# vliu15/speech-masters-thesis

Hardware: AMD Instinct MI355X
Metric: LJSpeech utterances/sec per VQ-VAE train step (higher is better)
Workload: dtype bf16

## Files before the change

speech-masters-thesis_amd/csrc/conv_common.h:

```cpp
#pragma once
#include <algorithm>
#include <cstdlib>

#include "smt_common.h"

namespace smt {

typedef __bf16 bf16x8 __attribute__((ext_vector_type(8)));
typedef __bf16 bf16x4 __attribute__((ext_vector_type(4)));
typedef short s16x4 __attribute__((ext_vector_type(4)));

__device__ __forceinline__ unsigned fmix32(unsigned h) {
  h ^= h >> 16; h *= 0x85EBCA6Bu; h ^= h >> 13; h *= 0xC2B2AE35u; h ^= h >> 16;
  return h;
}
__device__ __forceinline__ bool drop_keep(unsigned long long i, unsigned key, unsigned thresh16) {
  unsigned h = fmix32((unsigned)(i >> 1) * 0x9E3779B1u + key);
  unsigned bits = (h >> (16 * (unsigned)(i & 1))) & 0xFFFFu;
  return bits >= thresh16;
}

template <typename T> struct Tr;
template <> struct Tr<__bf16> {
  static constexpr int EPV = 8;
  static constexpr int CCH = 128;
  static constexpr int KC = 128;
  static constexpr int BM = 128;
};
template <> struct Tr<float> {
  static constexpr int EPV = 4;
  static constexpr int CCH = 64;
  static constexpr int KC = 64;
  static constexpr int BM = 64;
};

template <typename T, int EPV> struct Vec { T v[EPV]; } __attribute__((aligned(16)));

__device__ __forceinline__ unsigned pack_bf16x2(float lo, float hi) {
  typedef __bf16 bf16x2 __attribute__((ext_vector_type(2)));
  bf16x2 v = {(__bf16)lo, (__bf16)hi};
  return __builtin_bit_cast(unsigned, v);
}

typedef short s16x2v __attribute__((ext_vector_type(2)));
typedef unsigned short u16x2v __attribute__((ext_vector_type(2)));
__device__ __forceinline__ unsigned pk_relu_bf16(unsigned w) {
  return __builtin_bit_cast(unsigned, __builtin_elementwise_max(__builtin_bit_cast(s16x2v, w), s16x2v{0, 0}));
}
__device__ __forceinline__ unsigned pk_keep_mask(unsigned h, unsigned thr_m1) {
  u16x2v d = __builtin_elementwise_sub_sat(__builtin_bit_cast(u16x2v, h), __builtin_bit_cast(u16x2v, thr_m1));
  d = __builtin_elementwise_min(d, u16x2v{1, 1});
  return __builtin_bit_cast(unsigned, (u16x2v)(u16x2v{0, 0} - d));
}

__device__ __forceinline__ float gate_tanh(float x) {
  const float e = __builtin_amdgcn_exp2f(x * 2.885390081777927f);
  return 1.f - 2.f * __builtin_amdgcn_rcpf(e + 1.f);
}

__device__ __forceinline__ void lds_dma16(const void* gsrc, void* lds_dst_wave_base) {
  __builtin_amdgcn_global_load_lds((const void __attribute__((address_space(1)))*)gsrc,
                                   (void __attribute__((address_space(3)))*)lds_dst_wave_base, 16, 0, 0);
}

typedef int i32x4v __attribute__((ext_vector_type(4)));
__device__ __forceinline__ __amdgpu_buffer_rsrc_t ws_rsrc(const void* base, long long byte_off, unsigned bytes) {
  return __builtin_amdgcn_make_buffer_rsrc(const_cast<char*>(reinterpret_cast<const char*>(base)) + byte_off, 0, (int)bytes, 0x00020000);
}
__device__ __forceinline__ void ws_dma16(__amdgpu_buffer_rsrc_t rs, unsigned voff, void* lds_wave_base) {
  __builtin_amdgcn_raw_ptr_buffer_load_lds(rs, (__attribute__((address_space(3))) void*)lds_wave_base, 16, (int)voff, 0, 0, 0);
}
__device__ __forceinline__ bool wg_tile_run(int ntiles, int tiles_per_wg, int& wg, int& tile_begin, int& tile_end) {
  const int nwg = gridDim.x;
  wg = (blockIdx.x & 7) * (nwg >> 3) + (blockIdx.x >> 3);
  tile_begin = wg * tiles_per_wg;
  tile_end = min(ntiles, tile_begin + tiles_per_wg);
  return tile_begin < tile_end;
}

__device__ __forceinline__ void pair_up8(unsigned (&v)[8]) {
#pragma unroll
  for (int h2 = 0; h2 < 2; ++h2)
#pragma unroll
    for (int d = 0; d < 2; ++d) {
      auto sw = __builtin_amdgcn_permlane32_swap(v[4 * h2 + d], v[4 * h2 + 2 + d], false, false);
      v[4 * h2 + d] = sw[0]; v[4 * h2 + 2 + d] = sw[1];
    }
}
__device__ __forceinline__ void store_paired(const unsigned (&v)[8], __amdgpu_buffer_rsrc_t rs, unsigned vo) {
  __builtin_amdgcn_raw_buffer_store_b128(i32x4v{(int)v[0], (int)v[1], (int)v[2], (int)v[3]}, rs, (int)vo, 0, 0);
  __builtin_amdgcn_raw_buffer_store_b128(i32x4v{(int)v[4], (int)v[5], (int)v[6], (int)v[7]}, rs, (int)(vo + 32u), 0, 0);
}

struct UntrackedRsrc { i32x4v w; };
__device__ __forceinline__ UntrackedRsrc untracked_rsrc(const void* base, long long byte_off, unsigned bytes) {
  const unsigned long long a = reinterpret_cast<unsigned long long>(base) + (unsigned long long)byte_off;
  UntrackedRsrc r;
  r.w = i32x4v{__builtin_amdgcn_readfirstlane((int)(unsigned)a), __builtin_amdgcn_readfirstlane((int)((a >> 32) & 0xffffu)),
               __builtin_amdgcn_readfirstlane((int)bytes), 0x00020000};
  return r;
}
__device__ __forceinline__ void untracked_dma16(const UntrackedRsrc& rs, unsigned voff, const void* lds_wave_base) {
  const unsigned m0v = __builtin_amdgcn_readfirstlane(
      (int)(unsigned)reinterpret_cast<size_t>((__attribute__((address_space(3))) const void*)lds_wave_base));
  asm volatile("s_mov_b32 m0, %2\n\ts_nop 4\n\tbuffer_load_dwordx4 %0, %1, 0 offen lds" : : "v"(voff), "s"(rs.w), "s"(m0v) : "memory");
}

__device__ __forceinline__ i32x4v untracked_load16(const void* sbase, unsigned voff) {
  i32x4v v;
  asm volatile("s_nop 4\n\tglobal_load_dwordx4 %0, %1, %2" : "=v"(v) : "v"(voff), "s"(sbase) : "memory");
  return v;
}

typedef unsigned u32x2v __attribute__((ext_vector_type(2)));
__device__ __forceinline__ u32x2v untracked_load8(const void* sbase, unsigned voff) {
  u32x2v v;
  asm volatile("s_nop 4\n\tglobal_load_dwordx2 %0, %1, %2" : "=v"(v) : "v"(voff), "s"(sbase) : "memory");
  return v;
}

template <typename T> __device__ __forceinline__ void pin_v(T& x) { asm volatile("" : "+v"(x)); }
template <typename T, int N> __device__ __forceinline__ void pin_v(T (&a)[N]) {
#pragma unroll
  for (int i = 0; i < N; ++i) pin_v(a[i]);
}
template <int N, typename... R> __device__ __forceinline__ void vm_wait(R&... regs) {
  static_assert(0 <= N && N <= 63, "vmcnt is a 6-bit field on gfx9");
  asm volatile("s_waitcnt vmcnt(%0)" ::"n"(N) : "memory");
  (pin_v(regs), ...);
}
template <int N, typename... R> __device__ __forceinline__ void lgkm_wait(R&... regs) {
  static_assert(0 <= N && N <= 15, "lgkmcnt is a 4-bit field on gfx9");
  asm volatile("s_waitcnt lgkmcnt(%0)" ::"n"(N) : "memory");
  (pin_v(regs), ...);
}
template <int N, typename... R> __device__ __forceinline__ void vm_wait_or_drain(bool counted, R&... regs) {
  if (counted) vm_wait<N>();
  else vm_wait<0>();
  (pin_v(regs), ...);
}
template <int N, typename... R> __device__ __forceinline__ void step_end_wait(R&... regs) {
  __builtin_amdgcn_sched_barrier(0);
  vm_wait<N>(regs...);
}

__device__ __forceinline__ int scalar_load_i32(const int* ptr) {
  int v;
  asm volatile("s_nop 4\n\ts_load_dword %0, %1, 0x0\n\ts_waitcnt lgkmcnt(0)" : "=s"(v) : "s"(ptr) : "memory");
  return v;
}

struct ConvArgs {
  const void* x; const void* w; const float* bias; void* y; const void* res; const void* gate_h; void* y_act;
  const int* lens_in; const int* lens_out;
  long long x_bs, y_bs, res_bs, gh_bs, ya_bs;
  int ldx, ldy, ldr, ldgh, ldya;
  int B, Tin, Tout, Cin, Cout;
  int taps, stride, dil, pad;
  int out_stride, out_offset, Ty;
  int act_out, epi_act;
  unsigned drop_keys[8]; int site_width; unsigned drop_thresh16; float drop_scale;
  const unsigned* drop_keys_dev; int drop_keys_dev_stride;
  int tiles_per_batch;
  int rs;
  const void* x2; const void* w2; const float* bias2; const int* lens_in2; long long x2_bs; int ldx2;
  int dbg;
};

__device__ __forceinline__ unsigned site_key(const ConvArgs& p, int site) {
  return p.drop_keys_dev ? p.drop_keys_dev[(site & 7) * p.drop_keys_dev_stride] : p.drop_keys[site & 7];
}

struct WsPlan { int buf_bytes; size_t lds; int tiles_per_wg; dim3 grid; };
bool plan_conv_ws(ConvArgs& p, WsPlan& pl);
// ... 19 lines not shown
```

speech-masters-thesis_amd/csrc/conv_ws.hip:

```cpp
#include <algorithm>
#include <cstdlib>
#include <type_traits>

#include "smt_common.h"
#include "conv_common.h"

namespace smt {

#ifndef SMT_WS_STAMP
#define SMT_WS_STAMP 0
#endif
#if SMT_WS_STAMP
__device__ unsigned long long ws_dbg[256 * 8 * 8];
#define WS_T(var) const unsigned long long var = __builtin_readcyclecounter()
#define WS_ACC(k, a, b) do { if (lane == 0 && wg < 256) ws_dbg[(wg * 8 + wave) * 8 + (k)] += (b) - (a); } while (0)
#else
#define WS_T(var) do {} while (0)
#define WS_ACC(k, a, b) do {} while (0)
#endif
constexpr int WS_AGPR_TAPS = 8;
constexpr int WS_BM = 128, WS_BN = 128, WS_NT = 256, WS_EPI = 128 * 256;
constexpr int WS_KC = 128, WS_ROWB = WS_KC * 2, WS_KSTEPS = WS_KC / 16;

template <int I, int N, typename F>
__device__ __forceinline__ void static_for(F&& f) {
  if constexpr (I < N) {
    f(std::integral_constant<int, I>{});
    static_for<I + 1, N>(f);
  }
}


__device__ __forceinline__ bf16x8 ws_wfrag(const unsigned char* wrow, int kk, int hh, int co) {
  return *reinterpret_cast<const bf16x8*>(wrow + (((2 * kk + hh) ^ (co & 15)) << 4));
}

__device__ __forceinline__ void ws_decode(int tiles_per_batch, int rs, int tile, int& b, int& cls, int& t0) {
  const int bb = tile / tiles_per_batch;
  b = bb / rs; cls = bb - b * rs;
  t0 = (tile - bb * tiles_per_batch) * WS_BM;
}

__device__ __forceinline__ unsigned ws_tap_base(unsigned abase, int ar, int hh) { return abase + ar * WS_ROWB + ((hh ^ (ar & 15)) << 4); }
template <int NTAPS>
__device__ __forceinline__ unsigned ws_frag_addr(const unsigned (&tap_base)[NTAPS], int q) {
  return tap_base[q / WS_KSTEPS] ^ (32u * (q % WS_KSTEPS));
}

template <int MW>
__device__ __forceinline__ void ws_read_frags(bf16x8 (&afr)[MW], unsigned ap) {
#pragma unroll
  for (int i = 0; i < MW; ++i)
    asm volatile("ds_read_b128 %0, %1 offset:%2" : "=v"(afr[i]) : "v"(ap), "n"(i * 32 * WS_ROWB));
}
__device__ __forceinline__ void ws_first_use(f32x16& acc) { asm volatile("s_nop 4" : "+v"(acc)); }
__device__ __forceinline__ void ws_first_use(f32x16& acc0, f32x16& acc1) { asm volatile("s_nop 4" : "+v"(acc0), "+v"(acc1)); }
__device__ __forceinline__ void ws_mfma(f32x16& acc, const bf16x8& w, const bf16x8& a, bool w_in_agpr) {
  if (w_in_agpr) asm volatile("v_mfma_f32_32x32x16_bf16 %0, %1, %2, %0" : "+v"(acc) : "a"(w), "v"(a));
  else asm volatile("v_mfma_f32_32x32x16_bf16 %0, %1, %2, %0" : "+v"(acc) : "v"(w), "v"(a));
}
template <int MW>
__device__ __forceinline__ void ws_drain(f32x16 (&acc)[MW]) {
  static_assert(MW == 2 || MW == 4, "the drain names two or four accumulators");
#define WS_DRAIN_NOPS "s_nop 15\n\ts_nop 15\n\ts_nop 15\n\ts_nop 15"
  if constexpr (MW == 4) asm volatile(WS_DRAIN_NOPS : "+v"(acc[0]), "+v"(acc[1]), "+v"(acc[2]), "+v"(acc[3]));
  else asm volatile(WS_DRAIN_NOPS : "+v"(acc[0]), "+v"(acc[1]));
#undef WS_DRAIN_NOPS
}

template <int NTAPS, int MODE>
__global__ __launch_bounds__(WS_NT) void conv_ws_kernel(ConvArgs p, const __bf16* __restrict__ zero_page,
                                                        int tiles_per_wg, int buf_bytes) {
  const bool has_y = MODE == 0 ? (p.y != nullptr) : (MODE == 2);
  const bool has_act_out = MODE == 0 ? (p.act_out != 0) : (MODE == 1);
  const bool has_res = MODE == 0 ? (p.res != nullptr) : (MODE == 2);
  const bool has_epi_act = MODE == 0 ? (p.epi_act != 0) : (MODE == 2);
  typedef __bf16 T;
  constexpr int BM = WS_BM, BN = WS_BN, KC = WS_KC, NT = WS_NT, MW = BM / 32, ROWB = WS_ROWB;
  extern __shared__ __attribute__((aligned(1024))) unsigned char smem[];
  const int tid = threadIdx.x, lane = tid & 63, wave = tid >> 6;
  const int r = lane & 31, hh = lane >> 5;
  const int lrow = lane >> 4, lch = lane & 15;
  const int n0 = blockIdx.y * BN;
  const int rs = p.rs;

  int wg, tile_begin, tile_end;
  if (!wg_tile_run(p.tiles_per_batch * p.B * rs, tiles_per_wg, wg, tile_begin, tile_end)) return;

  unsigned char* lds_res = smem + 2 * (size_t)buf_bytes + wave * (WS_EPI / 4);
  unsigned char* lds_act = lds_res + WS_EPI;
  const unsigned lds_base = (unsigned)(uintptr_t)(__attribute__((address_space(3))) unsigned char*)smem;

  bf16x8 wfrag[NTAPS][KC / 16];
  {
    const int co = n0 + wave * 32 + r;
#pragma unroll
    for (int s = 0; s < NTAPS; ++s) {
      const unsigned char* wrow = reinterpret_cast<const unsigned char*>(p.w) + ((size_t)s * p.Cout + co) * ROWB;
#pragma unroll
      for (int kk = 0; kk < KC / 16; ++kk)
        wfrag[s][kk] = ws_wfrag(wrow, kk, hh, co);
    }
  }
  const int col0 = n0 + wave * 32 + 4 * hh;
  float bval[16];
// ... 135 lines not shown
        uint2 uv[4], rv[4];
#pragma unroll
        for (int g = 0; g < 4; ++g) {
          const int eoff = row * 64 + ((g ^ swz) << 4) + 8 * hh;
          uv[g] = *reinterpret_cast<const uint2*>(lds_act + eoff);
          rv[g] = *reinterpret_cast<const uint2*>(lds_res + eoff);
        }
        unsigned yp[8];
#pragma unroll
        for (int g = 0; g < 4; ++g) {
          const unsigned uvp[2] = {uv[g].x, uv[g].y}, rvp[2] = {rv[g].x, rv[g].y};
#pragma unroll
          for (int j = 0; j < 2; ++j) {
            const unsigned ypk = pack_bf16x2(acc[i][4 * g + 2 * j] + bval[4 * g + 2 * j], acc[i][4 * g + 2 * j + 1] + bval[4 * g + 2 * j + 1]);
            const float o0 = __builtin_bit_cast(float, ypk << 16), o1 = __builtin_bit_cast(float, ypk & 0xffff0000u);
            const float v0 = (uvp[j] & 0x7fffu) ? o0 * srow : 0.f, v1 = (uvp[j] & 0x7fff0000u) ? o1 * srow : 0.f;
            yp[2 * g + j] = pack_bf16x2(v0 + __builtin_bit_cast(float, rvp[j] << 16), v1 + __builtin_bit_cast(float, rvp[j] & 0xffff0000u));
          }
        }
        pair_up8(yp);
        store_paired(yp, ry, (unsigned)tc * pitch_y + (unsigned)hh * 16u);
      }
    } else {
#pragma unroll
    for (int i = 0; i < MW; ++i) {
      const int row = 32 * i + r;
      const int tc = t0 + row;
      const int ty = cls + rs * tc;
      const float keep_row = (ty >= len_out) ? 0.f : 1.f;
      const int swz = (row >> 2) & 3;
      unsigned yp[8], up[8];
      {
#pragma unroll
      for (int g = 0; g < 4; ++g) {
        float o[4];
#pragma unroll
        for (int k = 0; k < 4; ++k) o[k] = (float)(T)(acc[i][4 * g + k] + bval[4 * g + k]);
        const int eoff = row * 64 + ((g ^ swz) << 4) + 8 * hh;
        if (has_epi_act) {
          const bf16x4 uv = *reinterpret_cast<const bf16x4*>(lds_act + eoff);
#pragma unroll
          for (int k = 0; k < 4; ++k) o[k] = ((float)uv[k] != 0.f) ? o[k] * p.drop_scale : 0.f;
        }
        if (has_res) {
          const bf16x4 rv = *reinterpret_cast<const bf16x4*>(lds_res + eoff);
#pragma unroll
          for (int k = 0; k < 4; ++k) o[k] = fmaf(o[k], keep_row, (float)rv[k]);
        } else {
#pragma unroll
          for (int k = 0; k < 4; ++k) o[k] *= keep_row;
        }
        yp[2 * g] = pack_bf16x2(o[0], o[1]);
        yp[2 * g + 1] = pack_bf16x2(o[2], o[3]);
        if (has_act_out) {
          const int col = col0 + 8 * g;
          const int site = col / p.site_width;
          const unsigned key = site_key(p, site);
          const unsigned long long base = ((unsigned long long)b * p.Ty + ty) * p.site_width + (col - site * p.site_width);
#pragma unroll
          for (int k = 0; k < 4; k += 2) {
            const unsigned h = fmix32((unsigned)((base + k) >> 1) * 0x9E3779B1u + key);
            const bool k0 = (h & 0xFFFFu) >= p.drop_thresh16, k1 = (h >> 16) >= p.drop_thresh16;
            up[2 * g + (k >> 1)] = pack_bf16x2((k0 && o[k] > 0.f) ? o[k] * p.drop_scale : 0.f,
                                               (k1 && o[k + 1] > 0.f) ? o[k + 1] * p.drop_scale : 0.f);
          }
        }
      }
      }
      if (has_y) {
        pair_up8(yp);
        store_paired(yp, ry, (unsigned)tc * pitch_y + (unsigned)hh * 16u);
      }
      if (has_act_out) {
        pair_up8(up);
        store_paired(up, ru, (unsigned)tc * pitch_u + (unsigned)hh * 16u);
      }
    }
    }
    WS_T(c7);
    WS_ACC(0, c0, c1); WS_ACC(1, c1, c2); WS_ACC(3, c2, c4); WS_ACC(4, c4, c5); WS_ACC(5, c5, c6); WS_ACC(6, c6, c7); WS_ACC(7, c0, c0 + 1);
  }
}

template <int NTAPS>
__global__ __launch_bounds__(WS_NT) void conv_ws_pipe_kernel(ConvArgs p, const __bf16* __restrict__ zero_page,
                                                             int tiles_per_wg, int buf_bytes) {
  constexpr int BM = WS_BM, BN = WS_BN, KC = WS_KC, NT = WS_NT, MW = BM / 32, ROWB = WS_ROWB;
  constexpr int NSTEP = NTAPS * (KC / 16), NGAP = NSTEP * MW;
  constexpr int PH_UNIT = 12, PH_ROW = 4 * PH_UNIT + 2, PH_TILE = MW * PH_ROW;
  constexpr int AGPR_TAPS = NTAPS < 8 ? NTAPS : 8;
  static_assert(MW == 4, "four accumulators");
  extern __shared__ __attribute__((aligned(1024))) unsigned char smem[];
  const int tid = threadIdx.x, lane = tid & 63, wave = tid >> 6;
  const int r = lane & 31, hh = lane >> 5;
  const int lrow = lane >> 4, lch = lane & 15;
  const int n0 = blockIdx.y * BN;
  const int rs = p.rs;

  int wg, tile_begin, tile_end;
  if (!wg_tile_run(p.tiles_per_batch * p.B * rs, tiles_per_wg, wg, tile_begin, tile_end)) return;
  const unsigned lds_base = (unsigned)(uintptr_t)(__attribute__((address_space(3))) unsigned char*)smem;

  bf16x8 wfrag[NTAPS][KC / 16];
  {
    const int co = n0 + wave * 32 + r;
#pragma unroll
    for (int s = 0; s < NTAPS; ++s) {
      const unsigned char* wrow = reinterpret_cast<const unsigned char*>(p.w) + ((size_t)s * p.Cout + co) * ROWB;
#pragma unroll
      for (int kk = 0; kk < KC / 16; ++kk)
        wfrag[s][kk] = ws_wfrag(wrow, kk, hh, co);
    }
  }
  const int col0 = n0 + wave * 32 + 4 * hh;
  float bval[16];
#pragma unroll
  for (int e = 0; e < 16; ++e) bval[e] = p.bias ? p.bias[col0 + 8 * (e >> 2) + (e & 3)] : 0.f;
  unsigned keyg[4], cshalf[4];
#pragma unroll
  for (int g = 0; g < 4; ++g) {
    const int col = col0 + 8 * g;
    const int site = col / p.site_width;
    keyg[g] = site_key(p, site);
    cshalf[g] = (unsigned)(col - site * p.site_width) >> 1;
  }
  const int rows_in = BM + (NTAPS - 1) * p.dil;
  const int rows_pad = (rows_in + 3) & ~3;

  auto decode = [&](int tile, int& b, int& cls, int& t0) { ws_decode(p.tiles_per_batch, rs, tile, b, cls, t0); };
  const unsigned pitch_x = (unsigned)p.ldx * rs * 2u;
  const unsigned voff_a0 = (unsigned)(4 * wave + lrow) * pitch_x + (unsigned)((lch ^ ((4 * wave + lrow) & 15)) << 4);
  const int ngroups = rows_pad >> 2;
  auto stage_a = [&](int tile, int buf) {
    int b, cls, t0;
    decode(tile, b, cls, t0);
    const int len_full = p.lens_in ? min(scalar_load_i32(p.lens_in + b), p.Tin) : p.Tin;
    const int len_in = max(0, (len_full - cls + rs - 1) / rs);
    const __amdgpu_buffer_rsrc_t rx = ws_rsrc(p.x, ((long long)b * p.x_bs + (long long)cls * p.ldx) * 2, (unsigned)len_in * pitch_x);
    unsigned vo = voff_a0 + (unsigned)(t0 - p.pad) * pitch_x;
    unsigned char* dst = smem + (size_t)buf * buf_bytes + wave * 1024;
    for (int g = wave; g < ngroups; g += NT / 64) {
      ws_dma16(rx, vo, dst);
      vo += 16u * pitch_x; dst += 4096;
    }
  };

  unsigned pc[MW][8];
  int p_b = 0, p_cls = 0, p_t0 = 0, p_Tc = 0, p_len = 0;
  __amdgpu_buffer_rsrc_t p_ru = ws_rsrc(p.y_act, 0, 0);
  float o0 = 0.f, o1 = 0.f, o2 = 0.f, o3 = 0.f, u0 = 0.f, u1 = 0.f, u2 = 0.f, u3 = 0.f, keepf = 1.f;
  unsigned h0 = 0, h1 = 0, rh = 0, up[8];
  int ty = 0;
  auto fbits = [](unsigned v) { return __builtin_bit_cast(float, v); };
  auto epi = [&](auto M) {
    constexpr int m = decltype(M)::value;
    constexpr int i = m / PH_ROW, rem = m % PH_ROW;
    if constexpr (rem < 4 * PH_UNIT) {
      constexpr int g = rem / PH_UNIT, ph = rem % PH_UNIT;
      if constexpr (ph == 0) {
        if constexpr (g == 0) {
          const int tc = p_t0 + 32 * i + r;
          ty = (tc < p_Tc) ? p_cls + rs * tc : -1;
          keepf = (ty >= p_len) ? 0.f : 1.f;
          rh = (unsigned)((((unsigned long long)p_b * p.Ty + (unsigned)max(ty, 0)) * (unsigned)p.site_width) >> 1);
        }
      } else if constexpr (ph == 1) {
        o0 = fbits(pc[i][2 * g] << 16) * keepf; o1 = fbits(pc[i][2 * g] & 0xffff0000u) * keepf;
      } else if constexpr (ph == 2) {
        o2 = fbits(pc[i][2 * g + 1] << 16) * keepf; o3 = fbits(pc[i][2 * g + 1] & 0xffff0000u) * keepf;
      } else if constexpr (ph == 3) {
        h0 = (rh + cshalf[g]) * 0x9E3779B1u + keyg[g]; h1 = h0 + 0x9E3779B1u;
      } else if constexpr (ph == 4) {
        h0 ^= h0 >> 16; h0 *= 0x85EBCA6Bu; h1 ^= h1 >> 16; h1 *= 0x85EBCA6Bu;
      } else if constexpr (ph == 5) {
        h0 ^= h0 >> 13; h0 *= 0xC2B2AE35u; h1 ^= h1 >> 13; h1 *= 0xC2B2AE35u;
      } else if constexpr (ph == 6) {
        h0 ^= h0 >> 16; h1 ^= h1 >> 16;
      } else if constexpr (ph == 7) {
        u0 = ((h0 & 0xFFFFu) >= p.drop_thresh16 && o0 > 0.f) ? o0 * p.drop_scale : 0.f;
      } else if constexpr (ph == 8) {
        u1 = ((h0 >> 16) >= p.drop_thresh16 && o1 > 0.f) ? o1 * p.drop_scale : 0.f;
      } else if constexpr (ph == 9) {
        u2 = ((h1 & 0xFFFFu) >= p.drop_thresh16 && o2 > 0.f) ? o2 * p.drop_scale : 0.f;
      } else if constexpr (ph == 10) {
        u3 = ((h1 >> 16) >= p.drop_thresh16 && o3 > 0.f) ? o3 * p.drop_scale : 0.f;
      } else {
        up[2 * g] = pack_bf16x2(u0, u1); up[2 * g + 1] = pack_bf16x2(u2, u3);
      }
    } else if constexpr (rem == 4 * PH_UNIT) {
      pair_up8(up);
    } else {
      if (ty >= 0) {
        store_paired(up, p_ru, (unsigned)ty * ((unsigned)p.ldya * 2u) + (unsigned)hh * 16u);
      }
    }
  };

  stage_a(tile_begin, 0);
  vm_wait<0>();
  const int wave_s = __builtin_amdgcn_readfirstlane(wave);
#pragma unroll
  for (int i = 0; i < MW; ++i)
#pragma unroll
    for (int e = 0; e < 8; ++e) pc[i][e] = 0;
  for (int tile = tile_begin; tile < tile_end; ++tile) {
    const int buf = (tile - tile_begin) & 1;
    int b, cls, t0;
    decode(tile, b, cls, t0);
    WS_T(c0);
    __syncthreads();
    WS_T(c1);
    __amdgpu_buffer_rsrc_t rx_n = ws_rsrc(p.x, 0, 0);
    unsigned vo_in = 0;
    int n_in = 0;
    if (tile + 1 < tile_end) {
      int nb, ncls, nt0;
      decode(tile + 1, nb, ncls, nt0);
      const int len_full = p.lens_in ? min(scalar_load_i32(p.lens_in + nb), p.Tin) : p.Tin;
      const int len_in = max(0, (len_full - ncls + rs - 1) / rs);
      rx_n = ws_rsrc(p.x, ((long long)nb * p.x_bs + (long long)ncls * p.ldx) * 2, (unsigned)len_in * pitch_x);
      vo_in = voff_a0 + (unsigned)(nt0 - p.pad) * pitch_x;
      n_in = ngroups;
    }
    unsigned char* const dst_in = smem + (size_t)(buf ^ 1) * buf_bytes + wave_s * 1024;
    constexpr int WS_IN_SLOTS = 12, WS_IN_EVERY = 2;
    static_assert(WS_IN_SLOTS * WS_IN_EVERY <= NSTEP, "the pieces fit the tap loop");
    WS_T(c2);

    f32x16 acc[MW];
#pragma unroll
    for (int i = 0; i < MW; ++i)
#pragma unroll
      for (int e = 0; e < 16; ++e) acc[i][e] = 0.f;
    const unsigned abase = lds_base + (unsigned)buf * (unsigned)buf_bytes;
    unsigned tap_base[NTAPS];
#pragma unroll
    for (int s = 0; s < NTAPS; ++s) tap_base[s] = ws_tap_base(abase, r + s * p.dil, hh);
    auto frag_addr = [&](int q) -> unsigned { return ws_frag_addr(tap_base, q); };
    bf16x8 afr[2][MW];

    ws_read_frags(afr[0], frag_addr(0));
    static_for<0, NSTEP>([&](auto Q) {
      constexpr int q = decltype(Q)::value;
      if constexpr (q + 1 < NSTEP) {
        ws_read_frags(afr[(q + 1) & 1], frag_addr(q + 1));
        lgkm_wait<MW>();
      } else {
        lgkm_wait<0>();
      }
      static_for<0, MW>([&](auto I) {
        constexpr int i = decltype(I)::value;
        if constexpr (q == 0) ws_first_use(acc[i]);
        ws_mfma(acc[i], wfrag[q / (KC / 16)][q % (KC / 16)], afr[q & 1][i], q / (KC / 16) < AGPR_TAPS);
        if constexpr (i == 0 && q % WS_IN_EVERY == 0 && q / WS_IN_EVERY < WS_IN_SLOTS) {
          constexpr int j = q / WS_IN_EVERY;
          __builtin_amdgcn_sched_barrier(0);
          if (wave_s + 4 * j < n_in) ws_dma16(rx_n, vo_in + (unsigned)(16 * j) * pitch_x, dst_in + j * 4096);
          __builtin_amdgcn_sched_barrier(0);
        }
        if constexpr (4 * q + i < PH_TILE) {
          __builtin_amdgcn_sched_barrier(0);
          epi(std::integral_constant<int, 4 * q + i>{});
          __builtin_amdgcn_sched_barrier(0);
        }
      });
    });
    static_for<(NGAP < PH_TILE ? NGAP : PH_TILE), PH_TILE>(epi);
    ws_drain(acc);
    WS_T(c5);
    vm_wait<0>();
    WS_T(c6);
#pragma unroll
    for (int i = 0; i < MW; ++i)
#pragma unroll
      for (int e = 0; e < 16; e += 2) pc[i][e >> 1] = pack_bf16x2(acc[i][e] + bval[e], acc[i][e + 1] + bval[e + 1]);
    p_b = b; p_cls = cls; p_t0 = t0;
    p_ru = ws_rsrc(p.y_act, ((long long)b * p.ya_bs + n0 + wave_s * 32) * 2, (unsigned)p.Ty * ((unsigned)p.ldya * 2u));
    p_Tc = (p.Tout - cls + rs - 1) / rs;
    p_len = p.lens_out ? scalar_load_i32(p.lens_out + b) : 0x7fffffff;
    WS_T(c7);
    WS_ACC(0, c0, c1); WS_ACC(1, c1, c2); WS_ACC(4, c2, c5); WS_ACC(5, c5, c6); WS_ACC(6, c6, c7); WS_ACC(7, c0, c0 + 1);
  }
  static_for<0, PH_TILE>(epi);
}

constexpr int WS2_NT = 512;
constexpr int WS2_MAX_TAPS = 3;

template <int NTAPS, int MODE>
__global__ __launch_bounds__(WS2_NT) void conv_ws2_kernel(ConvArgs p, const __bf16* __restrict__ zero_page,
                                                          int tiles_per_wg, int buf_bytes) {
  constexpr int BM = WS_BM, BN = WS_BN, KC = WS_KC, MW = 2, ROWB = WS_ROWB;
  constexpr int NSTEP = NTAPS * (KC / 16), NG = 5;
  static_assert(MODE == 1 || MODE == 2, "two epilogues");
  constexpr int AGPR_TAPS = NTAPS < 4 ? NTAPS : 4;
  static_assert(NTAPS <= 5, "weights of more than five taps do not fit two waves per SIMD");
  extern __shared__ __attribute__((aligned(1024))) unsigned char smem[];
  const int tid = threadIdx.x, lane = tid & 63;
  const int wave = __builtin_amdgcn_readfirstlane(tid >> 6);
  const int cw = wave & 3, rhalf = wave >> 2;
  const int r = lane & 31, hh = lane >> 5;
  const int n0 = blockIdx.y * BN;
  const int rs = p.rs;

  int wg, tile_begin, tile_end;
  if (!wg_tile_run(p.tiles_per_batch * p.B * rs, tiles_per_wg, wg, tile_begin, tile_end)) return;

  float* lds_bias = reinterpret_cast<float*>(smem + 2 * (size_t)buf_bytes);
  unsigned char* lds_res = smem + 2 * (size_t)buf_bytes + 1024 + wave * (WS_EPI / 8);
  unsigned char* lds_act = lds_res + WS_EPI;
  const unsigned lds_base = (unsigned)(uintptr_t)(__attribute__((address_space(3))) unsigned char*)smem;
  if (tid < BN) lds_bias[tid] = p.bias ? p.bias[n0 + tid] : 0.f;

  bf16x8 wfrag[NTAPS][KC / 16];
  {
    const int co = n0 + cw * 32 + r;
#pragma unroll
    for (int s = 0; s < NTAPS; ++s) {
      const unsigned char* wrow = reinterpret_cast<const unsigned char*>(p.w) + ((size_t)s * p.Cout + co) * ROWB;
#pragma unroll
      for (int kk = 0; kk < KC / 16; ++kk)
        wfrag[s][kk] = ws_wfrag(wrow, kk, hh, co);
    }
  }
  const int col0 = n0 + cw * 32 + 4 * hh;
  const unsigned HC = 0x9E3779B1u;
  const unsigned swh = (unsigned)p.site_width >> 1;
  unsigned kc[4];
  unsigned rowh_lane = 0;
  const unsigned thr_m1 = (p.drop_thresh16 - 1u) * 0x00010001u;
  if (MODE == 1) {
#pragma unroll
    for (int g = 0; g < 4; ++g) {
      const int col = col0 + 8 * g;
      const int site = col / p.site_width;
      kc[g] = ((unsigned)(col - site * p.site_width) >> 1) * HC + site_key(p, site);
    }
    rowh_lane = HC * swh * (unsigned)(rs * r);
  }
  const int rows_in = BM + (NTAPS - 1) * p.dil;
  const int ngroups = (rows_in + 3) >> 2;

  const unsigned pitch_x = (unsigned)p.ldx * rs * 2u;
  unsigned voff_a[NG];
#pragma unroll
  for (int j = 0; j < NG; ++j) {
    const int row = 4 * (wave + 8 * j) + (lane >> 4);
    voff_a[j] = (unsigned)row * pitch_x + (unsigned)(((lane & 15) ^ (row & 15)) << 4);
  }
  const unsigned pitch_o = (MODE == 2 ? (unsigned)p.ldy : (unsigned)p.ldya) * rs * 2u;
  const unsigned voff_o = (unsigned)(64 * rhalf + r) * pitch_o + (unsigned)hh * 16u;
  const unsigned pitch_r = (unsigned)p.ldr * rs * 2u, pitch_g = (unsigned)p.ldgh * rs * 2u;
  const int elr = 64 * rhalf + (lane >> 2);
  const unsigned echunk = (unsigned)(((lane & 3) ^ ((lane >> 4) & 3)) << 4);

  auto decode = [&](int tile, int& b, int& cls, int& t0) { ws_decode(p.tiles_per_batch, rs, tile, b, cls, t0); };
  auto stage_a = [&](int tile, int buf) {
    int b, cls, t0;
    decode(tile, b, cls, t0);
    const int len_full = p.lens_in ? min(scalar_load_i32(p.lens_in + b), p.Tin) : p.Tin;
    const int len_in = max(0, (len_full - cls + rs - 1) / rs);
// ... 68 lines not shown
  vm_wait<0>();
  int pb = 0, pcls = 0, pt0 = 0, pTc = 0;
  for (int tile = tile_begin; tile < tile_end; ++tile) {
    const int buf = (tile - tile_begin) & 1;
    int b, cls, t0;
    decode(tile, b, cls, t0);
    const int Tc = (p.Tout - cls + rs - 1) / rs;
    WS_T(c0);
    __syncthreads();
    WS_T(c1);
    if (tile + 1 < tile_end) stage_a(tile + 1, buf ^ 1);
    WS_T(c2);
    if (rhalf == 1 && tile > tile_begin) epilogue(pb, pcls, pt0, pTc);
    WS_T(c3);
    if (MODE == 2) {
      stage_epi(p.res, p.res_bs, p.ldr, pitch_r, b, cls, t0, Tc, lds_res);
      stage_epi(p.gate_h, p.gh_bs, p.ldgh, pitch_g, b, cls, t0, Tc, lds_act);
    }
    WS_T(c4);
#pragma unroll
    for (int i = 0; i < MW; ++i)
#pragma unroll
      for (int e = 0; e < 16; ++e) acc[i][e] = 0.f;
    const unsigned abase = lds_base + (unsigned)buf * (unsigned)buf_bytes + (unsigned)(64 * rhalf) * ROWB;
    unsigned tap_base[NTAPS];
#pragma unroll
    for (int s = 0; s < NTAPS; ++s) {
      const int ar = r + s * p.dil;
      tap_base[s] = abase + ar * ROWB + ((hh ^ (ar & 15)) << 4);
    }
    auto frag_addr = [&](int q) -> unsigned { return ws_frag_addr(tap_base, q); };
    bf16x8 afr[3][MW];
#pragma unroll
    for (int q0 = 0; q0 < 2; ++q0) {
      const unsigned ap = frag_addr(q0);
      ws_read_frags(afr[q0], ap);
    }
    static_for<0, NSTEP>([&](auto Q) {
      constexpr int q = decltype(Q)::value;
      if constexpr (q + 2 < NSTEP) {
        const unsigned ap = frag_addr(q + 2);
        ws_read_frags(afr[(q + 2) % 3], ap);
        lgkm_wait<2 * MW>();
      } else if constexpr (q + 1 < NSTEP) {
        lgkm_wait<MW>();
      } else {
        lgkm_wait<0>();
      }
      static_assert(MW == 2, "two accumulators per wave");
      if constexpr (q == 0) ws_first_use(acc[0], acc[1]);
      ws_mfma(acc[0], wfrag[q / (KC / 16)][q % (KC / 16)], afr[q % 3][0], q / (KC / 16) < AGPR_TAPS);
      ws_mfma(acc[1], wfrag[q / (KC / 16)][q % (KC / 16)], afr[q % 3][1], q / (KC / 16) < AGPR_TAPS);
    });
    ws_drain(acc);
    WS_T(c5);
    vm_wait<0>();
    WS_T(c6);
    if (rhalf == 0) epilogue(b, cls, t0, Tc);
    WS_T(c7);
    WS_ACC(0, c0, c1); WS_ACC(1, c1, c2); WS_ACC(2, c2, c3); WS_ACC(3, c3, c4); WS_ACC(4, c4, c5); WS_ACC(5, c5, c6);
    WS_ACC(6, c6, c7); WS_ACC(7, c0, c0 + 1);
    pb = b; pcls = cls; pt0 = t0; pTc = Tc;
  }
  if (rhalf == 1) epilogue(pb, pcls, pt0, pTc);
}

#ifndef SMT_WS_AB
#define SMT_WS_AB 0
#endif

static int ws_min_tiles() {
  static const int v = getenv("SMT_WS_MIN_TILES") ? atoi(getenv("SMT_WS_MIN_TILES")) : 512;
  return v;
}

bool plan_conv_ws(ConvArgs& p, WsPlan& pl) {
  static const bool no_ws = getenv("SMT_CONV_NO_WS") != nullptr;
  const int tc_max = (p.Tout + p.rs - 1) / p.rs;
  const int rows_pad = (WS_BM + (p.taps - 1) * p.dil + 3) & ~3;
  const int buf_bytes = (int)align_up((size_t)std::max(rows_pad * 256, WS_BM * (WS_BN + 8) * 2), 1024);
  const size_t lds = 2 * (size_t)buf_bytes + 2 * WS_EPI;
  const int tpb = (tc_max + WS_BM - 1) / WS_BM;
  const long long ntiles = (long long)tpb * p.B * p.rs;
  if (no_ws || p.Cin != 128 || p.taps < 3 || p.taps > 9 || !(p.taps & 1) || lds > 160 * 1024 || ntiles < ws_min_tiles()) return false;
  p.tiles_per_batch = tpb;
  const int nwg = 256;
  pl.buf_bytes = buf_bytes; pl.lds = lds;
  pl.tiles_per_wg = (int)((ntiles + nwg - 1) / nwg);
  pl.grid = dim3((unsigned)nwg, (unsigned)(p.Cout / WS_BN));
  return true;
}

enum WsVariant { WS2_FWD, WS2_DGRAD, WS_PIPE, WS_MODE1, WS_MODE2, WS_GENERIC };
static WsVariant ws_variant(const ConvArgs& p) {
  const bool y = p.y != nullptr, ao = p.act_out != 0, res = p.res != nullptr, ea = p.epi_act != 0;
  const bool fwd = !y && ao && !res && !ea, dgrad = y && !ao && res && ea;
#if SMT_WS_AB
  static const bool no_ws2 = getenv("SMT_CONV_NO_WS2") != nullptr, no_pipe = getenv("SMT_CONV_NO_PIPE") != nullptr;
#else
  constexpr bool no_ws2 = false, no_pipe = false;
#endif
  if (p.taps <= WS2_MAX_TAPS && !no_ws2 && (fwd || dgrad)) return fwd ? WS2_FWD : WS2_DGRAD;
  if (fwd) return no_pipe ? WS_MODE1 : WS_PIPE;
  return dgrad ? WS_MODE2 : WS_GENERIC;
}

const char* conv_ws_variant_name(const ConvArgs& p) {
  switch (ws_variant(p)) {
    case WS2_FWD: case WS2_DGRAD: return "conv_ws2";
    case WS_PIPE: return "conv_ws_pipe";
    default: return "conv_ws";
  }
}

template <typename K>
static void launch_ws_kernel(K kernel, int nt, size_t lds, const ConvArgs& p, const WsPlan& pl, const void* zero_page, hipStream_t stream) {
  (void)hipFuncSetAttribute((const void*)kernel, hipFuncAttributeMaxDynamicSharedMemorySize, 160 * 1024);
  kernel<<<pl.grid, nt, lds, stream>>>(p, (const __bf16*)zero_page, pl.tiles_per_wg, pl.buf_bytes);
}

template <int NTAPS>
static void launch_ws(const ConvArgs& p, const WsPlan& pl, const void* zero_page, hipStream_t stream) {
  constexpr bool ws2 = NTAPS <= WS2_MAX_TAPS, one_wave = SMT_WS_AB || !ws2;
  const WsVariant v = ws_variant(p);
  if constexpr (ws2) {
    if (v == WS2_FWD) return launch_ws_kernel(conv_ws2_kernel<NTAPS, 1>, WS2_NT, 2 * (size_t)pl.buf_bytes + 1024, p, pl, zero_page, stream);
    if (v == WS2_DGRAD) return launch_ws_kernel(conv_ws2_kernel<NTAPS, 2>, WS2_NT, pl.lds + 1024, p, pl, zero_page, stream);
  }
  if constexpr (one_wave) {
    if (v == WS_PIPE) return launch_ws_kernel(conv_ws_pipe_kernel<NTAPS>, WS_NT, pl.lds, p, pl, zero_page, stream);
    if (v == WS_MODE2) return launch_ws_kernel(conv_ws_kernel<NTAPS, 2>, WS_NT, pl.lds, p, pl, zero_page, stream);
  }
  if constexpr (SMT_WS_AB) {
    if (v == WS_MODE1) return launch_ws_kernel(conv_ws_kernel<NTAPS, 1>, WS_NT, pl.lds, p, pl, zero_page, stream);
  }
  launch_ws_kernel(conv_ws_kernel<NTAPS, 0>, WS_NT, pl.lds, p, pl, zero_page, stream);
}

void launch_conv_ws(const ConvArgs& p, const WsPlan& pl, const void* zero_page, hipStream_t stream) {
  switch (p.taps) {
    case 3: return launch_ws<3>(p, pl, zero_page, stream);
    case 5: return launch_ws<5>(p, pl, zero_page, stream);
    case 7: return launch_ws<7>(p, pl, zero_page, stream);
    default: return launch_ws<9>(p, pl, zero_page, stream);
  }
}

}

using namespace smt;

#if SMT_WS_STAMP
extern "C" int smt_ws_debug_dump(unsigned long long* host, int n, int reset) {
  int rc = (int)hipMemcpyFromSymbol(host, HIP_SYMBOL(ws_dbg), sizeof(unsigned long long) * n);
  if (reset) { static unsigned long long z[256 * 8 * 8]; rc |= (int)hipMemcpyToSymbol(HIP_SYMBOL(ws_dbg), z, sizeof(z)); }
  return rc;
}
#endif
```

Baseline: 516.3.

## Spread pipelined-conv epilogue across MFMA gaps with constexpr cost-balanced schedule

Replaces the fixed one-epilogue-step-per-MFMA-gap interleave in the pipelined conv kernel with a compile-time schedule. The schedule packs dropout/activation epilogue steps into gaps by estimated cycle cost, so the trailing epilogue no longer runs after the tap loop. It also restructures the epilogue to precompute per-row hash and store offsets, and folds the length mask into the dropout threshold. Stores become branchless by pointing dead rows at an out-of-range offset, and input DMAs become branchless via zero-size buffer descriptors plus a dump LDS slot. The risks are more VGPR pressure, a schedule that rests on hand-estimated costs, and a new plan guard on the y_act size.

```diff
diff --git a/speech-masters-thesis_amd/csrc/conv_common.h b/speech-masters-thesis_amd/csrc/conv_common.h
--- a/speech-masters-thesis_amd/csrc/conv_common.h
+++ b/speech-masters-thesis_amd/csrc/conv_common.h
@@ -90,6 +90,10 @@
 __device__ __forceinline__ void store_paired(const unsigned (&v)[8], __amdgpu_buffer_rsrc_t rs, unsigned vo) {
   __builtin_amdgcn_raw_buffer_store_b128(i32x4v{(int)v[0], (int)v[1], (int)v[2], (int)v[3]}, rs, (int)vo, 0, 0);
   __builtin_amdgcn_raw_buffer_store_b128(i32x4v{(int)v[4], (int)v[5], (int)v[6], (int)v[7]}, rs, (int)(vo + 32u), 0, 0);
+}
+template <int H>
+__device__ __forceinline__ void store_paired_half(const unsigned (&v)[8], __amdgpu_buffer_rsrc_t rs, unsigned vo) {
+  __builtin_amdgcn_raw_buffer_store_b128(i32x4v{(int)v[4 * H], (int)v[4 * H + 1], (int)v[4 * H + 2], (int)v[4 * H + 3]}, rs, (int)(vo + 32u * H), 0, 0);
 }
 
 struct UntrackedRsrc { i32x4v w; };
diff --git a/speech-masters-thesis_amd/csrc/conv_ws.hip b/speech-masters-thesis_amd/csrc/conv_ws.hip
--- a/speech-masters-thesis_amd/csrc/conv_ws.hip
+++ b/speech-masters-thesis_amd/csrc/conv_ws.hip
@@ -21,6 +21,7 @@
 constexpr int WS_AGPR_TAPS = 8;
 constexpr int WS_BM = 128, WS_BN = 128, WS_NT = 256, WS_EPI = 128 * 256;
 constexpr int WS_KC = 128, WS_ROWB = WS_KC * 2, WS_KSTEPS = WS_KC / 16;
+constexpr unsigned WS_NO_ROW = 0xFFFFFF00u;
 
 template <int I, int N, typename F>
 __device__ __forceinline__ void static_for(F&& f) {
@@ -322,12 +323,52 @@
   }
 }
 
+constexpr int WS_PIPE_HDR = 3, WS_PIPE_UNIT = 10, WS_PIPE_ROW = WS_PIPE_HDR + 4 * WS_PIPE_UNIT + 3, WS_PIPE_STEPS = 4 * WS_PIPE_ROW;
+constexpr int WS_PIPE_SLOTS = 12, WS_PIPE_SLOT_EVERY = 2;
+constexpr int ws_pipe_step_cost(int m) {
+  const int rem = m % WS_PIPE_ROW;
+  if (rem < WS_PIPE_HDR) return rem == 0 ? 32 : rem == 1 ? 8 : 16;
+  if (rem < WS_PIPE_HDR + 4 * WS_PIPE_UNIT) {
+    constexpr int unit[WS_PIPE_UNIT] = {16, 24, 24, 24, 24, 8, 28, 28, 28, 28};
+    return unit[(rem - WS_PIPE_HDR) % WS_PIPE_UNIT];
+  }
+  return rem == WS_PIPE_ROW - 3 ? 16 : rem == WS_PIPE_ROW - 2 ? 20 : 4;
+}
+constexpr int ws_pipe_gap_base(int gap, int ngap) {
+  const int q = gap / 4, i = gap % 4;
+  int c = 0;
+  if (i == 3 && gap + 1 < ngap) c += 24;
+  if (q == 0 && i < 3) c += 38;
+  if (i == 0 && q % WS_PIPE_SLOT_EVERY == 0 && q / WS_PIPE_SLOT_EVERY < WS_PIPE_SLOTS) c += 24;
+  return c;
+}
+template <int NGAP>
+struct WsPipeSchedule { short first[NGAP + 1]; int limit; };
+template <int NGAP>
+constexpr WsPipeSchedule<NGAP> ws_pipe_schedule() {
+  WsPipeSchedule<NGAP> s{};
+  for (int limit = 24; limit <= 64; limit += 4) {
+    int m = 0;
+    for (int g = 0; g + 1 < NGAP; ++g) {
+      s.first[g] = (short)m;
+      int c = ws_pipe_gap_base(g, NGAP);
+      while (m < WS_PIPE_STEPS && c + ws_pipe_step_cost(m) <= limit) c += ws_pipe_step_cost(m++);
+    }
+    s.first[NGAP - 1] = (short)m;
+    s.first[NGAP] = (short)WS_PIPE_STEPS;
+    s.limit = limit;
+    if (m == WS_PIPE_STEPS) break;
+  }
+  return s;
+}
+
 template <int NTAPS>
 __global__ __launch_bounds__(WS_NT) void conv_ws_pipe_kernel(ConvArgs p, const __bf16* __restrict__ zero_page,
                                                              int tiles_per_wg, int buf_bytes) {
   constexpr int BM = WS_BM, BN = WS_BN, KC = WS_KC, NT = WS_NT, MW = BM / 32, ROWB = WS_ROWB;
   constexpr int NSTEP = NTAPS * (KC / 16), NGAP = NSTEP * MW;
-  constexpr int PH_UNIT = 12, PH_ROW = 4 * PH_UNIT + 2, PH_TILE = MW * PH_ROW;
+  constexpr int PH_HDR = WS_PIPE_HDR, PH_UNIT = WS_PIPE_UNIT, PH_ROW = WS_PIPE_ROW, PH_TILE = WS_PIPE_STEPS;
+  constexpr WsPipeSchedule<NGAP> SCHED = ws_pipe_schedule<NGAP>();
   constexpr int AGPR_TAPS = NTAPS < 8 ? NTAPS : 8;
   static_assert(MW == 4, "four accumulators");
   extern __shared__ __attribute__((aligned(1024))) unsigned char smem[];
@@ -356,13 +397,12 @@
   float bval[16];
 #pragma unroll
   for (int e = 0; e < 16; ++e) bval[e] = p.bias ? p.bias[col0 + 8 * (e >> 2) + (e & 3)] : 0.f;
-  unsigned keyg[4], cshalf[4];
+  unsigned csk[4];
 #pragma unroll
   for (int g = 0; g < 4; ++g) {
     const int col = col0 + 8 * g;
     const int site = col / p.site_width;
-    keyg[g] = site_key(p, site);
-    cshalf[g] = (unsigned)(col - site * p.site_width) >> 1;
+    csk[g] = ((unsigned)(col - site * p.site_width) >> 1) * 0x9E3779B1u + site_key(p, site);
   }
   const int rows_in = BM + (NTAPS - 1) * p.dil;
   const int rows_pad = (rows_in + 3) & ~3;
@@ -386,53 +426,60 @@
   };
 
   unsigned pc[MW][8];
-  int p_b = 0, p_cls = 0, p_t0 = 0, p_Tc = 0, p_len = 0;
+  int p_rem = 0, p_ty0 = 0, p_len = 0;
+  unsigned long long p_S = 0;
+  unsigned p_vo0 = 0;
   __amdgpu_buffer_rsrc_t p_ru = ws_rsrc(p.y_act, 0, 0);
-  float o0 = 0.f, o1 = 0.f, o2 = 0.f, o3 = 0.f, u0 = 0.f, u1 = 0.f, u2 = 0.f, u3 = 0.f, keepf = 1.f;
-  unsigned h0 = 0, h1 = 0, rh = 0, up[8];
+  const unsigned pitch_y = (unsigned)p.ldya * 2u;
+  const int rsr = rs * r;
+  const unsigned long long rsrW = (unsigned long long)(unsigned)rsr * (unsigned)p.site_width;
+  const unsigned rsrP = (unsigned)rsr * pitch_y + (unsigned)hh * 16u;
+  float o0 = 0.f, o1 = 0.f, o2 = 0.f, o3 = 0.f, u0 = 0.f, u1 = 0.f, u2 = 0.f, u3 = 0.f;
+  unsigned h0 = 0, h1 = 0, rh = 0, rhc = 0, thr = 0, vo_st = 0, up[8];
   int ty = 0;
   auto fbits = [](unsigned v) { return __builtin_bit_cast(float, v); };
   auto epi = [&](auto M) {
     constexpr int m = decltype(M)::value;
     constexpr int i = m / PH_ROW, rem = m % PH_ROW;
-    if constexpr (rem < 4 * PH_UNIT) {
-      constexpr int g = rem / PH_UNIT, ph = rem % PH_UNIT;
+    if constexpr (rem == 0) {
+      ty = (r < p_rem - 32 * i) ? p_ty0 + 32 * i * rs + rsr : -1;
+      thr = (ty >= p_len) ? 0x10000u : p.drop_thresh16;
+    } else if constexpr (rem == 1) {
+      rh = (unsigned)((p_S + (unsigned long long)(unsigned)(32 * i * rs) * (unsigned)p.site_width + rsrW) >> 1);
+    } else if constexpr (rem == 2) {
+      rhc = rh * 0x9E3779B1u;
+    } else if constexpr (rem < PH_HDR + 4 * PH_UNIT) {
+      constexpr int g = (rem - PH_HDR) / PH_UNIT, ph = (rem - PH_HDR) % PH_UNIT;
       if constexpr (ph == 0) {
-        if constexpr (g == 0) {
-          const int tc = p_t0 + 32 * i + r;
-          ty = (tc < p_Tc) ? p_cls + rs * tc : -1;
-          keepf = (ty >= p_len) ? 0.f : 1.f;
-          rh = (unsigned)((((unsigned long long)p_b * p.Ty + (unsigned)max(ty, 0)) * (unsigned)p.site_width) >> 1);
-        }
+        h0 = rhc + csk[g]; h1 = h0 + 0x9E3779B1u; h0 ^= h0 >> 16; h1 ^= h1 >> 16;
       } else if constexpr (ph == 1) {
-        o0 = fbits(pc[i][2 * g] << 16) * keepf; o1 = fbits(pc[i][2 * g] & 0xffff0000u) * keepf;
+        h0 *= 0x85EBCA6Bu; o0 = fbits(pc[i][2 * g] << 16); o1 = fbits(pc[i][2 * g] & 0xffff0000u);
       } else if constexpr (ph == 2) {
-        o2 = fbits(pc[i][2 * g + 1] << 16) * keepf; o3 = fbits(pc[i][2 * g + 1] & 0xffff0000u) * keepf;
+        h1 *= 0x85EBCA6Bu; o2 = fbits(pc[i][2 * g + 1] << 16); o3 = fbits(pc[i][2 * g + 1] & 0xffff0000u);
       } else if constexpr (ph == 3) {
-        h0 = (rh + cshalf[g]) * 0x9E3779B1u + keyg[g]; h1 = h0 + 0x9E3779B1u;
+        h0 ^= h0 >> 13; h0 *= 0xC2B2AE35u;
       } else if constexpr (ph == 4) {
-        h0 ^= h0 >> 16; h0 *= 0x85EBCA6Bu; h1 ^= h1 >> 16; h1 *= 0x85EBCA6Bu;
+        h1 ^= h1 >> 13; h1 *= 0xC2B2AE35u;
       } else if constexpr (ph == 5) {
-        h0 ^= h0 >> 13; h0 *= 0xC2B2AE35u; h1 ^= h1 >> 13; h1 *= 0xC2B2AE35u;
+        h0 ^= h0 >> 16; h1 ^= h1 >> 16;
       } else if constexpr (ph == 6) {
-        h0 ^= h0 >> 16; h1 ^= h1 >> 16;
+        u0 = ((h0 & 0xFFFFu) >= thr && o0 > 0.f) ? o0 * p.drop_scale : 0.f;
       } else if constexpr (ph == 7) {
-        u0 = ((h0 & 0xFFFFu) >= p.drop_thresh16 && o0 > 0.f) ? o0 * p.drop_scale : 0.f;
+        u1 = ((h0 >> 16) >= thr && o1 > 0.f) ? o1 * p.drop_scale : 0.f;
+        up[2 * g] = pack_bf16x2(u0, u1);
       } else if constexpr (ph == 8) {
-        u1 = ((h0 >> 16) >= p.drop_thresh16 && o1 > 0.f) ? o1 * p.drop_scale : 0.f;
-      } else if constexpr (ph == 9) {
-        u2 = ((h1 & 0xFFFFu) >= p.drop_thresh16 && o2 > 0.f) ? o2 * p.drop_scale : 0.f;
-      } else if constexpr (ph == 10) {
-        u3 = ((h1 >> 16) >= p.drop_thresh16 && o3 > 0.f) ? o3 * p.drop_scale : 0.f;
+        u2 = ((h1 & 0xFFFFu) >= thr && o2 > 0.f) ? o2 * p.drop_scale : 0.f;
       } else {
-        up[2 * g] = pack_bf16x2(u0, u1); up[2 * g + 1] = pack_bf16x2(u2, u3);
-      }
-    } else if constexpr (rem == 4 * PH_UNIT) {
+        u3 = ((h1 >> 16) >= thr && o3 > 0.f) ? o3 * p.drop_scale : 0.f;
+        up[2 * g + 1] = pack_bf16x2(u2, u3);
+      }
+    } else if constexpr (rem == PH_HDR + 4 * PH_UNIT) {
       pair_up8(up);
+    } else if constexpr (rem == PH_HDR + 4 * PH_UNIT + 1) {
+      vo_st = (ty >= 0) ? p_vo0 + (unsigned)(32 * i * rs) * pitch_y + rsrP : WS_NO_ROW;
+      store_paired_half<0>(up, p_ru, vo_st);
     } else {
-      if (ty >= 0) {
-        store_paired(up, p_ru, (unsigned)ty * ((unsigned)p.ldya * 2u) + (unsigned)hh * 16u);
-      }
+      store_paired_half<1>(up, p_ru, vo_st);
     }
   };
 
@@ -450,20 +497,22 @@
     WS_T(c0);
     __syncthreads();
     WS_T(c1);
-    __amdgpu_buffer_rsrc_t rx_n = ws_rsrc(p.x, 0, 0);
-    unsigned vo_in = 0;
+    const char* xb_n = reinterpret_cast<const char*>(p.x);
+    unsigned len_n = 0, vo_in = 0;
     int n_in = 0;
     if (tile + 1 < tile_end) {
       int nb, ncls, nt0;
       decode(tile + 1, nb, ncls, nt0);
       const int len_full = p.lens_in ? min(scalar_load_i32(p.lens_in + nb), p.Tin) : p.Tin;
       const int len_in = max(0, (len_full - ncls + rs - 1) / rs);
-      rx_n = ws_rsrc(p.x, ((long long)nb * p.x_bs + (long long)ncls * p.ldx) * 2, (unsigned)len_in * pitch_x);
+      xb_n += ((long long)nb * p.x_bs + (long long)ncls * p.ldx) * 2;
+      len_n = (unsigned)len_in * pitch_x;
       vo_in = voff_a0 + (unsigned)(nt0 - p.pad) * pitch_x;
       n_in = ngroups;
     }
     unsigned char* const dst_in = smem + (size_t)(buf ^ 1) * buf_bytes + wave_s * 1024;
-    constexpr int WS_IN_SLOTS = 12, WS_IN_EVERY = 2;
+    unsigned char* const dst_dump = smem + 2 * (size_t)buf_bytes + wave_s * 1024;
+    constexpr int WS_IN_SLOTS = WS_PIPE_SLOTS, WS_IN_EVERY = WS_PIPE_SLOT_EVERY;
     static_assert(WS_IN_SLOTS * WS_IN_EVERY <= NSTEP, "the pieces fit the tap loop");
     WS_T(c2);
 
@@ -492,20 +541,22 @@
         constexpr int i = decltype(I)::value;
         if constexpr (q == 0) ws_first_use(acc[i]);
         ws_mfma(acc[i], wfrag[q / (KC / 16)][q % (KC / 16)], afr[q & 1][i], q / (KC / 16) < AGPR_TAPS);
-        if constexpr (i == 0 && q % WS_IN_EVERY == 0 && q / WS_IN_EVERY < WS_IN_SLOTS) {
+        constexpr bool dma_gap = i == 0 && q % WS_IN_EVERY == 0 && q / WS_IN_EVERY < WS_IN_SLOTS;
+        if constexpr (dma_gap) {
           constexpr int j = q / WS_IN_EVERY;
           __builtin_amdgcn_sched_barrier(0);
-          if (wave_s + 4 * j < n_in) ws_dma16(rx_n, vo_in + (unsigned)(16 * j) * pitch_x, dst_in + j * 4096);
+          const bool want = wave_s + 4 * j < n_in;
+          ws_dma16(ws_rsrc(xb_n, 0, want ? len_n : 0u), vo_in + (unsigned)(16 * j) * pitch_x, want ? dst_in + j * 4096 : dst_dump);
           __builtin_amdgcn_sched_barrier(0);
         }
-        if constexpr (4 * q + i < PH_TILE) {
+        __builtin_amdgcn_sched_barrier(0);
+        static_for<SCHED.first[4 * q + i], SCHED.first[4 * q + i + 1]>([&](auto M) {
           __builtin_amdgcn_sched_barrier(0);
-          epi(std::integral_constant<int, 4 * q + i>{});
+          epi(M);
           __builtin_amdgcn_sched_barrier(0);
-        }
+        });
       });
     });
-    static_for<(NGAP < PH_TILE ? NGAP : PH_TILE), PH_TILE>(epi);
     ws_drain(acc);
     WS_T(c5);
     vm_wait<0>();
@@ -514,9 +565,11 @@
     for (int i = 0; i < MW; ++i)
 #pragma unroll
       for (int e = 0; e < 16; e += 2) pc[i][e >> 1] = pack_bf16x2(acc[i][e] + bval[e], acc[i][e + 1] + bval[e + 1]);
-    p_b = b; p_cls = cls; p_t0 = t0;
-    p_ru = ws_rsrc(p.y_act, ((long long)b * p.ya_bs + n0 + wave_s * 32) * 2, (unsigned)p.Ty * ((unsigned)p.ldya * 2u));
-    p_Tc = (p.Tout - cls + rs - 1) / rs;
+    p_ru = ws_rsrc(p.y_act, ((long long)b * p.ya_bs + n0 + wave_s * 32) * 2, (unsigned)p.Ty * pitch_y);
+    p_rem = (p.Tout - cls + rs - 1) / rs - t0;
+    p_ty0 = cls + rs * t0;
+    p_S = ((unsigned long long)b * p.Ty + (unsigned)p_ty0) * (unsigned)p.site_width;
+    p_vo0 = (unsigned)p_ty0 * pitch_y;
     p_len = p.lens_out ? scalar_load_i32(p.lens_out + b) : 0x7fffffff;
     WS_T(c7);
     WS_ACC(0, c0, c1); WS_ACC(1, c1, c2); WS_ACC(4, c2, c5); WS_ACC(5, c5, c6); WS_ACC(6, c6, c7); WS_ACC(7, c0, c0 + 1);
@@ -751,7 +804,8 @@
   const size_t lds = 2 * (size_t)buf_bytes + 2 * WS_EPI;
   const int tpb = (tc_max + WS_BM - 1) / WS_BM;
   const long long ntiles = (long long)tpb * p.B * p.rs;
-  if (no_ws || p.Cin != 128 || p.taps < 3 || p.taps > 9 || !(p.taps & 1) || lds > 160 * 1024 || ntiles < ws_min_tiles()) return false;
+  const bool ya_ok = !p.y_act || (unsigned long long)p.Ty * (unsigned)p.ldya * 2ull < WS_NO_ROW;
+  if (no_ws || p.Cin != 128 || p.taps < 3 || p.taps > 9 || !(p.taps & 1) || lds > 160 * 1024 || ntiles < ws_min_tiles() || !ya_ok) return false;
   p.tiles_per_batch = tpb;
   const int nwg = 256;
   pl.buf_bytes = buf_bytes; pl.lds = lds;
```

New measurement: 515.7 (median of 2 runs). Within noise of the previous version (-0.1%).
